# felixyu7/perceiver-io-1

Hardware: AMD Instinct MI355X
Metric: samples/sec (whole node) IMDB MLM seq_len=512 at 1/2/4/8 MI355X (higher is better)
Workload: dtype bf16; 1 GPU; mlm256; model=perceiver-io-mlm latents=256x64 layers=3x(1+6) vocab=10003, global_batch=64, seq_len=512, parallelism=dp1, backend=hip, graph=True, allreduce_in_graph=False, bucket_update=False

## Files before the change

### perceiver_io_amd/csrc/attention.hip

```cpp
#include "common.h"

namespace pio {

constexpr int KT = 64;

template <int D, int NWV>
__global__ __launch_bounds__(64 * NWV) void attn_fwd_kernel(AttnArgs a, uint16_t* __restrict__ O,
                                                            float* __restrict__ LSE, float* __restrict__ Opart,
                                                            float* __restrict__ MLpart, int nsplit,
                                                            int tiles_per_split) {
  constexpr int LDK = D + 8;
  constexpr int LDV = (D < 32 ? 32 : D) + 8;
  constexpr int NT = (D < 32) ? 1 : D / 32;
  constexpr int KS = D / 16;
  constexpr int CH = D / 8;
  constexpr int NTH = 64 * NWV;
  constexpr int NST0 = 4 * NTH / (KT * CH);
  constexpr int NST = NST0 >= 4 ? 4 : (NST0 >= 1 ? NST0 : 1);
  constexpr int NI = (NST * KT * CH + NTH - 1) / NTH;
  constexpr bool PF = NI <= 4;
  __shared__ __attribute__((aligned(16))) uint16_t sK[NST * KT * LDK];
  __shared__ __attribute__((aligned(16))) uint16_t sV[NST * KT * LDV + 64];

  const int w = wave_id(), l = lane_id(), r = l & 31, hh = l >> 5;
  const Blk3 blk = xcd_block3();
  const int h = blk.y;
  const int b = blk.z / nsplit, split = blk.z % nsplit;
  const int q0 = (blk.x * NWV + w) * 32;
  const int qi = q0 + r;
  const uint32_t dkey = a.drop_thresh ? drop_key(a.seedp, a.site, 2u) : 0u;
  const int qc = qi < a.Nq ? qi : a.Nq - 1;

  bf16x8 qf[KS];
  {
    const uint16_t* qp = a.q + (long long)b * a.q_bs + (long long)qc * a.q_rs + h * D + 8 * hh;
#pragma unroll
    for (int s = 0; s < KS; ++s) qf[s] = *reinterpret_cast<const bf16x8*>(qp + 16 * s);
  }

  const bool ones_den = D < 32 && !a.drop_thresh;
  if (D < 32) {
    const short pv = ones_den ? (short)0x3F80 : (short)0;
    const bf16x8 pad8 = {pv, pv, pv, pv, pv, pv, pv, pv};
    for (int i = threadIdx.x; i < NST * KT; i += NTH)
      *reinterpret_cast<bf16x8*>(sV + i * LDV + 16) = pad8, *reinterpret_cast<bf16x8*>(sV + i * LDV + 24) = pad8;
// ... 298 lines not shown
  bool kpad = false;
  if constexpr (KM) {
    const unsigned char* kmp = (a.kmask && kin) ? a.kmask + (long long)b * a.Nk + key
                                                : reinterpret_cast<const unsigned char*>(kZero32B);
    const unsigned char kmv = *kmp;
    kpad = (kmv != 0) | !kin;
  }

  const int HD = a.H * D;
  const bool vec_out = ((((uintptr_t)dq | (uintptr_t)dk | (uintptr_t)dv) & 15) == 0) &&
                       (((dq_bs | dk_bs | dv_bs) & 3) == 0) && (((dq_rs | dk_rs | dv_rs) & 3) == 0);
  const uint16_t* kbp = a.k + (long long)b * a.k_bs + h * D;
  const uint16_t* vbp = a.v + (long long)b * a.v_bs + h * D;
  const uint16_t* qbp = a.q + (long long)b * a.q_bs + h * D;
  const uint16_t* dobp = dO + (long long)b * a.Nq * HD + h * D;
  const int nqt_all = (a.Nq + 31) / 32;
  const int qt_begin = qsplit * q_tiles_per_split;
  const int nqt = min(nqt_all, qt_begin + q_tiles_per_split);

  bf16x8 qreg[NI];
  float lreg = 0.f;
  bool lq_out = false;
  auto fetch = [&](int qt0) {
    const int q00 = qt0 * 32;
#pragma unroll
    for (int i = 0; i < NI; ++i) {
      const int c = threadIdx.x + NTH * i, isdo = c >= NQS * 32 * CH, cc = isdo ? c - NQS * 32 * CH : c;
      const int qq = q00 + cc / CH, col = (cc % CH) * 8;
      const bool ok = c < NQS * 64 * CH && qq < a.Nq;
      const uint16_t* p = !ok ? reinterpret_cast<const uint16_t*>(kZero32B)
                              : (isdo ? dobp + (long long)qq * HD + col : qbp + (long long)qq * a.q_rs + col);
      qreg[i] = *reinterpret_cast<const bf16x8*>(p);
    }
    {
      const int t = threadIdx.x < NQS * 64 ? threadIdx.x : 0;
      const int isd = t >= NQS * 32, qq = q00 + (isd ? t - NQS * 32 : t);
      const long long idx = ((long long)b * a.Nq + qq) * a.H + h;
      const bool ok = qq < a.Nq;
      lreg = *(!ok ? kZero32B : (isd ? delta + idx : LSE + idx));
      lq_out = !ok && !isd;
    }
  };
  bf16x8 kf[KS], vf[KS];
#pragma unroll
  for (int s = 0; s < KS; ++s) {
    kf[s] = *reinterpret_cast<const bf16x8*>(kbp + (long long)kc * a.k_rs + 16 * s + 8 * hh);
    vf[s] = *reinterpret_cast<const bf16x8*>(vbp + (long long)kc * a.v_rs + 16 * s + 8 * hh);
  }
  fetch(qt_begin);
  if (D < 32) {
    for (int i = threadIdx.x; i < KB; i += NTH) {
      *reinterpret_cast<bf16x8*>(sK + i * LD + 16) = bf16x8{0, 0, 0, 0, 0, 0, 0, 0};
      *reinterpret_cast<bf16x8*>(sK + i * LD + 24) = bf16x8{0, 0, 0, 0, 0, 0, 0, 0};
// ... 110 lines not shown
    lds_sync();
    PIO_TS(4 + 4 * ((qt0 - qt_begin) / NQS));
    if constexpr (D == 16 && NW == 8 && (NQS == 4 || NQS == 2)) {
      const int j = w % NQS, mh = w / NQS, g = l >> 4;
      if (mh < 2 && qt0 + j < nqt) {
        const uint16_t* tS = sdS + j * KB * LDS_;
        f32x4 a0 = f32x4{0.f, 0.f, 0.f, 0.f}, a1 = f32x4{0.f, 0.f, 0.f, 0.f};
#pragma unroll
        for (int k0 = 0; k0 < KB; k0 += 64) {
          a0 = mfma16(frag16_tr(tS, LDS_, 16 * mh, k0), frag16_tr(sK, LD, 0, k0), a0);
          a1 = mfma16(frag16_tr(tS, LDS_, 16 * mh, k0 + 32), frag16_tr(sK, LD, 0, k0 + 32), a1);
        }
#pragma unroll
        for (int i = 0; i < 4; ++i) {
          const int qq = (qt0 + j) * 32 + 16 * mh + 4 * g + i;
          if (qq < a.Nq) {
            const long long di = (long long)b * dq_bs + (long long)qq * dq_rs + h * D + (l & 15);
            const float v = (a0[i] + a1[i]) * a.scale;
            if constexpr (OBF) reinterpret_cast<uint16_t*>(dq)[di] = f2bf(v);
            else if (dq_atomic) atomicAdd(dq + di, v);
            else dq[di] = v;
          }
        }
      }
    } else if (w < NQS && qt0 + w < nqt) {
      const uint16_t* tS = sdS + w * KB * LDS_;
#pragma unroll
      for (int t = 0; t < NT; ++t) {
        f32x16 dq_acc = f32x16{}, dq_acc2 = f32x16{};
#pragma unroll
        for (int k0 = 0; k0 < KB; k0 += 32) {
          dq_acc = mfma32(frag_ks(tS, LDS_, 0, k0), frag_ks(sK, LD, 32 * t, k0), dq_acc);
          dq_acc2 = mfma32(frag_ks(tS, LDS_, 0, k0 + 16), frag_ks(sK, LD, 32 * t, k0 + 16), dq_acc2);
        }
        dq_acc += dq_acc2;
        if (dq_atomic || !vec_out || D > 32) {
#pragma unroll
          for (int i = 0; i < 16; ++i) {
            const int dd = 32 * t + r, qq = (qt0 + w) * 32 + acc_row(i, hh);
            if (dd < D && qq < a.Nq) {
              float* dst = dq + (long long)b * dq_bs + (long long)qq * dq_rs + h * D + dd;
              const float v = dq_acc[i] * a.scale;
              if (dq_atomic) atomicAdd(dst, v);
              else *dst = v;
            }
          }
        } else {
          float* sE = reinterpret_cast<float*>(sdS + w * KB * LDS_);
          constexpr int LDE = D + 4;
#pragma unroll
          for (int i = 0; i < 16; ++i)
            if (r < D) sE[acc_row(i, hh) * LDE + r] = dq_acc[i] * a.scale;
          constexpr int CPR = D / 4;
#pragma unroll
          for (int c = l; c < 32 * CPR; c += 64) {
            const int qq = (qt0 + w) * 32 + c / CPR, col = (c % CPR) * 4;
            if (qq < a.Nq)
              *reinterpret_cast<float4*>(dq + (long long)b * dq_bs + (long long)qq * dq_rs + h * D + col) =
                  *reinterpret_cast<const float4*>(sE + (c / CPR) * LDE + col);
          }
        }
      }
    }
    PIO_TS(5 + 4 * ((qt0 - qt_begin) / NQS));
  }
  PIO_TS(40);
  if constexpr (D <= 32 && 2 * KB * (D + 4) * 4 <= NQS * KB * LDS_ * 2) {
    if (vec_out && nqs == 1) {
      constexpr int LDE = D + 4, CPR = D / 4;
      float* sE = reinterpret_cast<float*>(sdS);
      lds_sync();
#pragma unroll
// ... 295 lines not shown
```

### perceiver_io_amd/csrc/binding.cpp

```cpp
#include <torch/extension.h>
#include <ATen/hip/HIPContext.h>
#include <hip/hip_runtime.h>

#include "host_api.h"

#include <tuple>
#include <unordered_map>
#include <vector>

using torch::Tensor;
using OptT = c10::optional<Tensor>;

namespace {
hipStream_t stream() { return at::hip::getCurrentHIPStream(); }

#ifndef PIO_CHECKS
#define PIO_CHECKS 0
#endif
int64_t check_errors(bool reset) {
  return (int64_t)(pio::check_errors_elementwise(reset) | pio::check_errors_optim(reset) |
                   pio::check_errors_mlm_head(reset) | pio::check_errors_mlm_select(reset) |
                   pio::check_errors_ce_head(reset) | pio::check_errors_topk_head(reset) |
                   pio::check_errors_rowgemm(reset) | pio::check_errors_pixel_head(reset) |
                   pio::check_errors_soft_ce_head(reset) | pio::check_errors_augment(reset) |
// ... 78 lines not shown
    const Tensor& m = *kmask;
    CHECK_CUDA(m);
    TORCH_CHECK(m.scalar_type() == torch::kBool || m.scalar_type() == torch::kUInt8, "key mask must be bool/uint8");
    TORCH_CHECK(m.is_contiguous() && m.size(0) == a.B && m.size(1) == a.Nk, "key mask must be (B, Nk) contiguous");
    a.kmask = reinterpret_cast<const uint8_t*>(m.data_ptr());
  }
  a.scale = (float)scale;
  a.scale_log2 = (float)(scale * 1.4426950408889634);
  const pio::DropCfg d = make_drop(seed, site, dropout_p);
  a.drop_thresh = d.thresh;
  a.drop_scale = d.scale;
  a.seedp = d.seed;
  a.site = d.site;
  return a;
}
}

std::vector<Tensor> attn_fwd(Tensor q, Tensor k, Tensor v, OptT kmask, int64_t H, int64_t D, double scale,
                             double dropout_p, OptT seed, int64_t nsplit, int64_t site) {
  auto a = make_args(q, k, v, kmask, (int)H, (int)D, scale, dropout_p, seed, site);
  auto opts = q.options();
  Tensor O = torch::empty({a.B, a.Nq, H * D}, opts.dtype(torch::kBFloat16));
  Tensor L = torch::empty({a.B, a.Nq, H}, opts.dtype(torch::kFloat32));
  Tensor Op, ML;
  float* opp = nullptr; float* mlp = nullptr;
  if (nsplit > 1) {
    Op = torch::empty({nsplit, a.B, a.Nq, H, D}, opts.dtype(torch::kFloat32));
    ML = torch::empty({nsplit, a.B, a.Nq, H, 2}, opts.dtype(torch::kFloat32));
    opp = Op.data_ptr<float>(); mlp = ML.data_ptr<float>();
  }
  pio::attn_fwd_launch(a, (int)D, bfp_mut(O), L.data_ptr<float>(), opp, mlp, (int)std::max<int64_t>(1, nsplit), stream());
  return {O, L};
}

std::tuple<OptT, OptT> attn_weights(Tensor q, Tensor k, OptT kmask, Tensor lse, int64_t H, int64_t D, double scale,
// ... 15 lines not shown
    if (nchunks > 1) part = torch::empty({a.B, nchunks, a.Nk}, opts);
  }
  pio::attn_weights_launch(a, (int)D, f32p(lse), want_avg ? avg->data_ptr<float>() : nullptr,
                           want_mass ? mass->data_ptr<float>() : nullptr,
                           part.defined() ? part.data_ptr<float>() : nullptr, nchunks, stream());
  return {avg, mass};
}

namespace {
pio::SlabJob make_job(const OptT& slab, std::vector<Tensor>& dsts, const std::vector<int64_t>& offs);
}

std::vector<Tensor> attn_bwd(Tensor q, Tensor k, Tensor v, OptT kmask, Tensor o, Tensor dO, Tensor lse, OptT delta_in,
                             int64_t H, int64_t D, double scale, double dropout_p, OptT seed, OptT dq_out,
                             OptT dk_out, OptT dv_out, bool kv_accumulate, int64_t site, bool dq_zeroed,
                             bool kv_zeroed, OptT job_slab, std::vector<Tensor> job_dsts, std::vector<int64_t> job_offs) {
  auto a = make_args(q, k, v, kmask, (int)H, (int)D, scale, dropout_p, seed, site);
  const pio::SlabJob job = make_job(job_slab, job_dsts, job_offs);
  TORCH_CHECK(dO.is_contiguous() && o.is_contiguous(), "O / dO must be contiguous (B, Nq, H*D)");
  auto f32 = q.options().dtype(torch::kFloat32);
  if (dq_out.has_value() && dq_out->scalar_type() == torch::kBFloat16) {
    TORCH_CHECK(dk_out.has_value() && dv_out.has_value() && dk_out->scalar_type() == torch::kBFloat16 &&
                    dv_out->scalar_type() == torch::kBFloat16 && delta_in.has_value() && !kv_accumulate,
                "bf16 attn_bwd outputs: dq/dk/dv all bf16, delta given, no accumulation");
    Tensor dq = *dq_out, dk = *dk_out, dv = *dv_out;
    TORCH_CHECK(dq.stride(2) == 1 && dk.stride(2) == 1 && dv.stride(2) == 1, "dq/dk/dv need unit inner stride");
    Tensor delta = *delta_in;
    TORCH_CHECK(delta.is_contiguous() && delta.numel() == (int64_t)a.B * a.Nq * H, "delta must be (B, Nq, H)");
    CHECK_DT(delta, torch::kFloat32);
    if (pio::attn_bwd_bf16_ok(a, (int)D)) {
      pio::attn_bwd_bf16_launch(a, (int)D, bfp(dO), f32p(lse), delta.data_ptr<float>(), bfp_mut(dq), dq.stride(0),
                                (int)dq.stride(1), bfp_mut(dk), dk.stride(0), (int)dk.stride(1), bfp_mut(dv),
                                dv.stride(0), (int)dv.stride(1), job, stream());
    } else {
      if (job.slab) pio::slab_reduce_launch(job, stream());
      std::vector<Tensor> nd;
      auto r = attn_bwd(q, k, v, kmask, o, dO, lse, delta_in, H, D, scale, dropout_p, seed, c10::nullopt, c10::nullopt,
                        c10::nullopt, false, site, false, false, c10::nullopt, nd, {});
      dq.copy_(r[0]); dk.copy_(r[1]); dv.copy_(r[2]);
    }
    return {dq, dk, dv};
  }
  if (job.slab) pio::slab_reduce_launch(job, stream());
  Tensor dq = dq_out.has_value() ? *dq_out : torch::empty({a.B, a.Nq, H * D}, f32);
  Tensor dk = dk_out.has_value() ? *dk_out : torch::empty({a.B, a.Nk, H * D}, f32);
  Tensor dv = dv_out.has_value() ? *dv_out : torch::empty({a.B, a.Nk, H * D}, f32);
  TORCH_CHECK(dq.stride(2) == 1 && dk.stride(2) == 1 && dv.stride(2) == 1, "dq/dk/dv need unit inner stride");
  TORCH_CHECK(dq.size(0) == a.B && dq.stride(0) == a.Nq * dq.stride(1), "dq must be batch-dense");
  CHECK_DT(dq, torch::kFloat32); CHECK_DT(dk, torch::kFloat32); CHECK_DT(dv, torch::kFloat32);
  Tensor delta;
  if (delta_in.has_value()) {
    delta = *delta_in;
    TORCH_CHECK(delta.is_contiguous() && delta.numel() == (int64_t)a.B * a.Nq * H, "delta must be (B, Nq, H)");
    CHECK_DT(delta, torch::kFloat32);
  } else {
    delta = torch::empty({a.B, a.Nq, H}, f32);
  }
  auto rows3 = [](Tensor& t) { return pio::Rows3{t.data_ptr<float>(), t.stride(0), (int)t.stride(1)}; };
  pio::AttnBwdArgs b{};
  b.a = a;
  b.O = bfp(o);
  b.dO = bfp(dO);
  b.LSE = f32p(lse);
  b.delta = delta.data_ptr<float>();
// ... 888 lines not shown
  const int d = like.get_device();
  auto it = tickets.find(d);
  if (it == tickets.end()) it = tickets.emplace(d, torch::zeros({kCeTickets}, like.options().dtype(torch::kInt32))).first;
  return it->second;
}
constexpr int64_t kCeRowBlockTickets = 4096;
static Tensor& ce_rb_tickets(const Tensor& like) {
  static std::unordered_map<int, Tensor> tickets;
  const int d = like.get_device();
  auto it = tickets.find(d);
  if (it == tickets.end())
    it = tickets.emplace(d, torch::zeros({kCeRowBlockTickets}, like.options().dtype(torch::kInt32))).first;
  return it->second;
}

std::vector<Tensor> mlm_select(Tensor labels, int64_t cap, int64_t gcap, OptT sticky, OptT queries) {
  CHECK_DT(labels, torch::kInt64);
  TORCH_CHECK(labels.dim() == 2 && labels.is_contiguous(), "labels must be (B, L) contiguous");
  const int B = (int)labels.size(0), L = (int)labels.size(1);
  TORCH_CHECK(cap > 0 && cap <= L && gcap > 0 && B > 0, "bad capacities");
  auto i64 = labels.options();
  Tensor idx_b = torch::empty({B, cap}, i64), lab_b = torch::empty({B, cap}, i64);
  Tensor count = torch::empty({B}, i64.dtype(torch::kInt32));
  Tensor gidx = torch::empty({gcap}, i64), glab = torch::empty({gcap}, i64);
  Tensor total = torch::empty({1}, i64.dtype(torch::kFloat32)), ovf = torch::empty({1}, i64.dtype(torch::kBool));
  const float* P = nullptr;
  float* qp = nullptr;
  int C = 0;
  Tensor q;
  if (queries.has_value()) {
    CHECK_DT(*queries, torch::kFloat32);
    TORCH_CHECK(queries->dim() == 2 && queries->is_contiguous() && queries->size(0) >= L && queries->size(1) % 4 == 0 &&
                    queries->get_device() == labels.get_device(),
                "mlm_select: queries must be a contiguous fp32 (>= L, C) array, C % 4 == 0, on the labels' device");
    C = (int)queries->size(1);
    P = queries->data_ptr<float>();
    q = torch::empty({B, cap, C}, queries->options());
    qp = q.data_ptr<float>();
  }
  pio::mlm_select_launch(labels.data_ptr<int64_t>(), B, L, (int)cap, (int)gcap, idx_b.data_ptr<int64_t>(),
                         lab_b.data_ptr<int64_t>(), count.data_ptr<int>(), gidx.data_ptr<int64_t>(),
                         glab.data_ptr<int64_t>(), total.data_ptr<float>(), ovf.data_ptr<bool>(),
                         sticky.has_value() ? sticky->data_ptr<bool>() : nullptr, P, C, qp, stream());
  std::vector<Tensor> out{idx_b, lab_b, gidx, glab, total, ovf};
  if (queries.has_value()) out.push_back(q);
  return out;
}

static const int64_t* opt_idx(const OptT& idx, int64_t n) {
  if (!idx.has_value()) return nullptr;
  CHECK_DT(*idx, torch::kInt64);
  TORCH_CHECK(idx->is_contiguous() && idx->numel() == n, "ce: idx must hold one source row per row");
  return idx->data_ptr<int64_t>();
}

std::vector<Tensor> ce_fwd(Tensor h, OptT idx, Tensor labels, Tensor w, Tensor bias, Tensor count, OptT zero_out,
                           bool count_labels) {
  TORCH_CHECK(h.is_contiguous() && w.is_contiguous() && labels.is_contiguous() && bias.is_contiguous());
  CHECK_DT(labels, torch::kInt64);
  CHECK_DT(h, torch::kFloat32);
// ... 1220 lines not shown
  pio::attn_fwd_pe_launch(a, stream());
  pio::attn_combine_launch(a.Opart, a.MLpart, bfp_mut(o), lse.data_ptr<float>(), ns, (long long)B * Nq * H, 32, stream());
  return {o, lse};
}

void set_deterministic(bool on) { g_det = on; }
bool get_deterministic() { return g_det; }

PYBIND11_MODULE(TORCH_EXTENSION_NAME, m) {
  m.def("set_deterministic", &set_deterministic);
  m.def("check_errors", &check_errors, py::arg("reset") = true);
  m.def("checked_build", &checked_build);
  m.def("get_deterministic", &get_deterministic);
  m.doc() = "Perceiver IO CDNA4 (gfx950) kernels";
  m.def("attn_fwd", &attn_fwd, py::arg("q"), py::arg("k"), py::arg("v"), py::arg("kmask"), py::arg("H"), py::arg("D"),
        py::arg("scale"), py::arg("dropout_p"), py::arg("seed"), py::arg("nsplit"), py::arg("site") = 0);
  m.def("attn_bwd", &attn_bwd, py::arg("q"), py::arg("k"), py::arg("v"), py::arg("kmask"), py::arg("o"), py::arg("dO"),
        py::arg("lse"), py::arg("delta_in"), py::arg("H"), py::arg("D"), py::arg("scale"), py::arg("dropout_p"),
        py::arg("seed"), py::arg("dq_out"), py::arg("dk_out"), py::arg("dv_out"), py::arg("kv_accumulate") = false,
        py::arg("site") = 0, py::arg("dq_zeroed") = false, py::arg("kv_zeroed") = false,
        py::arg("job_slab") = py::none(), py::arg("job_dsts") = std::vector<Tensor>{},
        py::arg("job_offs") = std::vector<int64_t>{});
  m.def("attn_weights", &attn_weights, py::arg("q"), py::arg("k"), py::arg("kmask"), py::arg("lse"), py::arg("H"),
        py::arg("D"), py::arg("scale"), py::arg("want_avg"), py::arg("want_mass"));
  m.def("attn_bwd_zero_plan", &pio::attn_bwd_zero_plan, py::arg("B"), py::arg("H"), py::arg("Nq"), py::arg("Nk"),
        py::arg("D"));
  m.def("ln_linear_fwd", &ln_linear_fwd, py::arg("x"), py::arg("lnw"), py::arg("lnb"), py::arg("eps"), py::arg("w"),
        py::arg("bias"), py::arg("act"), py::arg("res"), py::arg("out_bf16"), py::arg("save_stats"),
        py::arg("pe") = py::none(), py::arg("kin") = -1, py::arg("pe_index") = py::none());
  m.def("post_attn_fwd", &post_attn_fwd, py::arg("o"), py::arg("x"), py::arg("wo"), py::arg("bo"), py::arg("g2"),
        py::arg("be2"), py::arg("eps"), py::arg("w1"), py::arg("b1"), py::arg("w2"), py::arg("b2"),
        py::arg("seed") = py::none(), py::arg("site") = 0, py::arg("p") = 0.0);
  m.def("sa_layer_fwd", &sa_layer_fwd, py::arg("qkv"), py::arg("x"), py::arg("N"), py::arg("scale"), py::arg("wo"),
        py::arg("bo"), py::arg("g2"), py::arg("be2"), py::arg("eps"), py::arg("w1"), py::arg("b1"), py::arg("w2"),
        py::arg("b2"), py::arg("lnw") = py::none(), py::arg("lnb") = py::none(), py::arg("wq") = py::none(),
        py::arg("bq") = py::none(), py::arg("seed") = py::none(), py::arg("site") = 0, py::arg("p") = 0.0);
  m.def("sb_fwd", &sb_fwd, py::arg("x"), py::arg("params"), py::arg("scale"), py::arg("eps"),
// ... 23 lines not shown
        py::arg("seed") = py::none(), py::arg("site") = 0, py::arg("p") = 0.0, py::arg("zero_out") = py::none());
  m.def("ln_linear_bwd", &ln_linear_bwd, py::arg("g"), py::arg("w"), py::arg("x"), py::arg("mean"), py::arg("rstd"),
        py::arg("lnw"), py::arg("lnb"), py::arg("dres"), py::arg("need_dx"), py::arg("dlnw"), py::arg("dlnb"),
        py::arg("dW"), py::arg("db"), py::arg("pe") = py::none(), py::arg("kin") = -1, py::arg("slab") = false,
        py::arg("job_slab") = py::none(), py::arg("job_dsts") = std::vector<Tensor>(),
        py::arg("job_offs") = std::vector<int64_t>(), py::arg("dx_out") = py::none(), py::arg("pe_index") = py::none());
  m.def("text_kv_fwd", &text_kv_fwd, py::arg("ids"), py::arg("E"), py::arg("P"), py::arg("scale"), py::arg("eps"),
        py::arg("la"), py::arg("lb"));
  m.def("text_kv_bwd", &text_kv_bwd, py::arg("ga"), py::arg("gb"), py::arg("x"), py::arg("mean"), py::arg("rstd"),
        py::arg("la"), py::arg("lb"), py::arg("grads"), py::arg("slab") = false, py::arg("job_slab") = py::none(),
        py::arg("job_dsts") = std::vector<Tensor>(), py::arg("job_offs") = std::vector<int64_t>());
  m.def("wgrad", &wgrad, py::arg("g"), py::arg("a"), py::arg("amode"), py::arg("mean"), py::arg("rstd"), py::arg("lnw"),
        py::arg("lnb"), py::arg("rows_per_wg"), py::arg("dW"), py::arg("db"), py::arg("pe") = py::none(),
        py::arg("kin") = -1, py::arg("pe_index") = py::none());
  m.def("mlm_select", &mlm_select, py::arg("labels"), py::arg("cap"), py::arg("gcap"), py::arg("sticky") = py::none(),
        py::arg("queries") = py::none());
  m.def("index_add_rows", &index_add_rows);
  m.def("gather_rows", &gather_rows, py::arg("src"), py::arg("idx"));
  m.def("batch_sum2", &batch_sum2, py::arg("a"), py::arg("b"), py::arg("ob_acc") = py::none());
  m.def("pixel_ce_fwd", &pixel_ce_fwd);
  m.def("pixel_ce_bwd", &pixel_ce_bwd);
  m.def("pixel_seg_fwd", &pixel_seg_fwd);
  m.def("pixel_seg_bwd", &pixel_seg_bwd);
  m.def("pixel_predict", &pixel_predict, py::arg("h"), py::arg("w"), py::arg("b"), py::arg("qidx"), py::arg("qvalid"),
        py::arg("Q"), py::arg("npix"), py::arg("labels") = py::none());
  m.def("nonzero_compact", &nonzero_compact, py::arg("img"), py::arg("cap"), py::arg("segs") = 0, py::arg("tile") = 0);
  m.def("event_compact", &event_compact, py::arg("img"), py::arg("lab"), py::arg("words"), py::arg("key_cap"),
        py::arg("query_cap"), py::arg("wmask"), py::arg("ncls"), py::arg("segs") = 0, py::arg("tile") = 0);
  m.def("stage_step", &stage_step, py::arg("dsts"), py::arg("srcs"), py::arg("hyper_dst") = py::none(),
        py::arg("hyper") = std::vector<double>{}, py::arg("seed_dst") = py::none(),
        py::arg("seeds") = std::vector<int64_t>{});
// ... 75 lines not shown
```

### perceiver_io_amd/csrc/host_api.h

```cpp
#pragma once
#include <stdint.h>

#include <hip/hip_runtime_api.h>

namespace pio {


struct AttnArgs {
  const uint16_t* q; long long q_bs; int q_rs;
  const uint16_t* k; long long k_bs; int k_rs;
  const uint16_t* v; long long v_bs; int v_rs;
  const uint8_t* kmask;
  int B, H, Nq, Nk;
  float scale_log2;
  float scale;
  uint32_t drop_thresh;
  float drop_scale;
  const int64_t* seedp;
  uint32_t site;
};

struct DropCfg {
  const int64_t* seed;
  uint32_t site;
  uint32_t thresh;
  float scale;
};

constexpr int kMaxSlabSegs = 16;
constexpr int kSlabColsPerBlock = 1024;
struct SlabJob {
  const float* slab;
  int S, P, nbx, nblk;
  int det;
// ... 423 lines not shown
```

### perceiver_io_amd/ops/emulation.py

```python
from __future__ import annotations

import math
import torch
import torch.nn.functional as F

LOG2E = 1.4426950408889634


def _bf(x):
    return x.to(torch.bfloat16).to(torch.float32)


M32 = 0xFFFFFFFF


def _u32(x):
    return x & M32


def hash3(a, b, c):
    h = _u32(_u32(a * 0x9E3779B1) ^ _u32(b + 0x7F4A7C15))
    h = h ^ _u32(c * 0x85EBCA77)
    h = _u32((h ^ (h >> 15)) * 0x2C1B3C6D)
    h = _u32((h ^ (h >> 12)) * 0x297A2D39)
# ... 246 lines not shown
def _qkv(q, k, v, H, D):
    B = max(q.shape[0], k.shape[0])
    qf = q[:, :, : H * D].float().expand(B, -1, -1).reshape(B, q.shape[1], H, D).permute(0, 2, 1, 3)
    kf = k[:, :, : H * D].float().reshape(B, k.shape[1], H, D).permute(0, 2, 1, 3)
    vf = v[:, :, : H * D].float().reshape(B, v.shape[1], H, D).permute(0, 2, 1, 3)
    return B, qf, kf, vf


def _scores(qf, kf, kmask, scale):
    s = torch.matmul(qf, kf.transpose(-1, -2)) * scale
    if kmask is not None:
        s = s.masked_fill(kmask.view(kmask.shape[0], 1, 1, -1).bool(), float("-inf"))
    return s


def attn_fwd(q, k, v, kmask, H, D, scale, dropout_p, seed, nsplit, site=0):
    B, qf, kf, vf = _qkv(q, k, v, H, D)
    s = _scores(qf, kf, kmask, scale)
    lse = torch.logsumexp(s, -1)
    p = torch.exp(s - lse[..., None])
    p = torch.nan_to_num(p, nan=0.0)
    if dropout_p > 0:
        p = p * attn_drop_mask(seed, site, B, H, q.shape[1], k.shape[1], dropout_p, q.device)
    o = torch.matmul(_bf(p), vf)
    lse2 = torch.where(torch.isfinite(lse), lse * LOG2E, torch.full_like(lse, float("inf")))
    o = o.permute(0, 2, 1, 3).reshape(B, q.shape[1], H * D).to(torch.bfloat16)
    return o, lse2.permute(0, 2, 1).contiguous()


def attn_weights(q, k, kmask, lse, H, D, scale, want_avg, want_mass):
    if not (want_avg or want_mass):
        raise ValueError("attn_weights: at least one of avg / mass must be requested")
    B, qf, kf, _ = _qkv(q, k, k, H, D)
    s = torch.matmul(qf, kf.transpose(-1, -2)) * scale
    if lse is not None:
        l2 = lse.float().permute(0, 2, 1).unsqueeze(-1)
        l2 = torch.where(torch.isfinite(l2), l2, torch.full_like(l2, float("inf")))
        p = torch.exp2(s * LOG2E - l2)
        if kmask is not None:
            p = p.masked_fill(kmask.view(B, 1, 1, -1).bool(), 0.0)
    else:
        if kmask is not None:
            s = s.masked_fill(kmask.view(B, 1, 1, -1).bool(), float("-inf"))
        p = torch.nan_to_num(torch.softmax(s, -1), nan=0.0)
    avg = p.sum(1) * (1.0 / H)
    return (avg if want_avg else None), (avg.sum(1) if want_mass else None)


def attn_bwd(q, k, v, kmask, o, dO, lse, delta_in, H, D, scale, dropout_p, seed, dq_out, dk_out, dv_out,
             kv_accumulate=False, site=0, dq_zeroed=False, kv_zeroed=False, job_slab=None, job_dsts=(), job_offs=()):
    _run_job(job_slab, job_dsts, job_offs)
    B, qf, kf, vf = _qkv(q, k, v, H, D)
    s = _scores(qf, kf, kmask, scale)
    l2 = lse.permute(0, 2, 1)
    p = torch.exp2(s * LOG2E - l2[..., None])
    p = torch.nan_to_num(p, nan=0.0)
    dof = dO.float().reshape(B, -1, H, D).permute(0, 2, 1, 3)
    if delta_in is not None:
        delta = delta_in.float().reshape(B, -1, H).permute(0, 2, 1)[..., None]
    else:
        of = o.float().reshape(B, -1, H, D).permute(0, 2, 1, 3)
        delta = (dof * of).sum(-1, keepdim=True)
    dp = torch.matmul(dof, vf.transpose(-1, -2))
    if dropout_p > 0:
        m = attn_drop_mask(seed, site, B, H, q.shape[1], k.shape[1], dropout_p, q.device)
        ds = p * (dp * m - delta)
        pd = p * m
    else:
        ds = p * (dp - delta)
        pd = p
    dq = torch.matmul(ds, kf) * scale
    dk = torch.matmul(ds.transpose(-1, -2), qf) * scale
    dv = torch.matmul(pd.transpose(-1, -2), dof)

    def merge(t):
        return t.permute(0, 2, 1, 3).reshape(B, t.shape[2], H * D)

# ... 118 lines not shown
        return d + dres if dres is not None else d
    return None


def wgrad(g, a, amode, mean, rstd, lnw, lnb, rows_per_wg, dW, db=None, pe=None, kin=-1, pe_index=None):
    af = _split_x(a, pe, kin if kin >= 0 else a.shape[1], pe_index)
    if amode == 1:
        af = (af - mean[:, None]) * rstd[:, None] * lnw + lnb
    elif amode == 2:
        af = F.gelu(af)
    _acc(dW, _bf(g.float()).t() @ _bf(af))
    if db is not None:
        _acc(db, g.float().sum(0))


def mlm_select(labels, cap, gcap, sticky=None, queries=None):
    B, L = labels.shape
    sel = labels != -100
    pos = torch.cumsum(sel.to(torch.int64), 1) - 1
    idx_b = (torch.arange(cap, device=labels.device) % L).repeat(B, 1)
    lab_b = torch.full((B, cap), -100, dtype=torch.int64, device=labels.device)
    keep = sel & (pos < cap)
    rows = torch.arange(B, device=labels.device)[:, None].expand(B, L)
    cols = torch.arange(L, device=labels.device).expand(B, L)
    idx_b[rows[keep], pos[keep]] = cols[keep]
    lab_b[rows[keep], pos[keep]] = labels[keep]
    count = sel.sum(1)
    n = count.clamp(max=cap)
    slot_ok = torch.arange(cap, device=labels.device)[None, :] < n[:, None]
    flat = torch.nonzero(slot_ok.reshape(-1)).reshape(-1)
    gidx = torch.zeros(gcap, dtype=torch.int64, device=labels.device)
    glab = torch.full((gcap,), -100, dtype=torch.int64, device=labels.device)
    m = min(gcap, flat.numel())
    gidx[:m] = flat[:m]
    glab[:m] = lab_b.reshape(-1)[flat[:m]]
    total = count.sum().float().reshape(1)
    ovf = ((count > cap).any() | (n.sum() > gcap)).reshape(1)
    if sticky is not None:
        sticky.logical_or_(ovf.reshape(sticky.shape))
    if queries is not None:
        return idx_b, lab_b, gidx, glab, total, ovf, queries.index_select(0, idx_b.reshape(-1)).view(B, cap, -1)
    return idx_b, lab_b, gidx, glab, total, ovf


def _ce_rows(h, idx):
    return h if idx is None else h.index_select(0, idx)


def ce_fwd(h, idx, labels, w, bias, count, zero_out=None, count_labels=False):
    if zero_out is not None:
        zero_out.zero_()
    if count_labels:
        count.reshape(-1)[0] = (labels >= 0).sum()
    logits = _bf(_ce_rows(h, idx).float()) @ _bf(w.float()).t() + bias
    lse = torch.logsumexp(logits, -1)
    valid = labels >= 0
    picked = logits.gather(1, labels.clamp(min=0)[:, None])[:, 0]
# ... 939 lines not shown
```

### perceiver_io_amd/ops/fused.py

```python
from __future__ import annotations

import math
import os
from dataclasses import dataclass
from typing import List, Optional

import torch

from . import emulation, ext
from ..parallel.reducer import bucket_ready_point

EPS = 1e-5
WGRAD_SLAB = True
BF16_DQKV = True
ATTN_SLAB = True
CHAIN_ATT = True
TALL_ROWS = 1 << 17


def kernels(t: torch.Tensor):
    return ext.require() if t.is_cuda else emulation


class WeightCache:
# ... 363 lines not shown
        C, H = spec.C, spec.heads
        D = C // H
        scale = 1.0 / math.sqrt(D)
        wq, wkv, wo, w1, w2 = bw
        if spec.cross:
            g_q, b_q, g_kv, b_kv = ps[0:4]
            rest = ps[5:] if spec.packed else ps[7:]
        else:
            g_q, b_q = ps[0:2]
            rest = ps[3:]
        bin_, _, bo, g2, be2, _, b1, _, b2 = rest
        Bq, Nq = x_q.shape[0], x_q.shape[1]
        xq2 = x_q.reshape(Bq * Nq, C)
        if not xq2.is_contiguous():
            xq2 = xq2.contiguous()
        if spec.cross:
            B, M = x_kv.shape[0], x_kv.shape[1]
            xkv2 = x_kv.reshape(B * M, x_kv.shape[2])
            hq = _LOOKAHEAD["have_q"]
            if hq is not None and hq[4] is g_q and hq[0].data_ptr() == xq2.data_ptr() and hq[0].numel() == xq2.numel():
                q, mean_q, rstd_q = hq[1:4]
                _LOOKAHEAD["have_q"] = None
                ctx.q_handoff = True
            else:
                q, mean_q, rstd_q = K.ln_linear_fwd(xq2, g_q, b_q, EPS, wq, bin_[:C], 0, None, True, True)
            key = id(ps[0])
            ent = src.entries.get(key) if src is not None else None
            ctx.kv_owner = ent is None or bool(ent.pop("claim", False))
            if ent is None:
                kv_sb = False
# ... 39 lines not shown
                k3, v3 = kv3[:, :, :C], kv3[:, :, C:]
        else:
            B = Bq
            qkv, mean_q, rstd_q = K.ln_linear_fwd(xq2, g_q, b_q, EPS, wq, bin_, 0, None, True, True)
            qkv3 = qkv.view(B, Nq, 3 * C)
            q3, k3, v3 = qkv3[:, :, :C], qkv3[:, :, C:2 * C], qkv3[:, :, 2 * C:]
            xkv2 = kv = mean_kv = rstd_kv = None
        from .attention import pick_splits

        imp = ent.get("implicit") if spec.cross else None
        if imp is not None:
            P, pes, pesq, wt, kin = imp
            o, lse = K.attn_fwd_pe(q3, P, xkv2, pes, pesq, wt, H, scale, kin, EPS, 0)
        else:
            nsplit = pick_splits(B, H, Nq, k3.shape[1], p_attn > 0)
            o, lse = K.attn_fwd(q3, k3, v3, kmask, H, D, scale, p_attn, seed, nsplit)
        o2 = o.view(B * Nq, C)
        nxt, _LOOKAHEAD["want"] = _LOOKAHEAD["want"], None
        want_pa, _LOOKAHEAD["want_pa"] = _LOOKAHEAD["want_pa"], None
        if (want_pa and spec.cross and nxt is None and p_attn == 0.0 and Nq == 32 and H == 4 and Bq in (1, B)
                and o2.is_contiguous()):
            z = torch.empty((B * Nq, C), device=o2.device, dtype=torch.float32)
            _LOOKAHEAD["have_pa"] = dict(key=z.data_ptr(), ctx=ctx, pre=[o2, xq2, wo, bo, g2, be2, w1, b1, w2, b2],
                                         ps=(rest[1], bo, g2, be2, rest[5], b1, rest[7], b2))
            ctx.pa_key = z.data_ptr()
            y = m2 = r2 = u = torch.empty(0, device=o2.device)
        elif nxt is not None and spec.cross:
            z, y, m2, r2, u, qkv_n, mean_n, rstd_n = K.post_attn_ln_linear_fwd(
                o2, xq2, wo, bo, g2, be2, EPS, w1, b1, w2, b2, nxt[0], nxt[1], nxt[2], nxt[3], seed=seed, p=p_attn)
            _LOOKAHEAD["have"] = (z, qkv_n, mean_n, rstd_n, nxt[0])
            ctx.lookahead_z = z.data_ptr()
# ... 117 lines not shown
                if imp is not None:
                    P, pes, pesq, wt, kin = imp
                    K.attn_bwd_pe_implicit(qx, P, pes, pesq, wt, do.view(B, Nq, C), lse, delta3, xkv2, dq, ent["pe_D"],
                                           ent["pe_part"], H, scale, kin, EPS, acc, ent["pe_bsplit"],
                                           dq_zeroed=dq_pre is not None, d_zeroed=d_pre is not None)
                else:
                    K.attn_bwd_pe(qx, kv, do.view(B, Nq, C), lse, delta3, mean_kv, rstd_kv, xkv2, dq, ent["pe_D"],
                                  ent["pe_part"], H, scale, acc, ent["pe_bsplit"], dq_zeroed=dq_pre is not None,
                                  d_zeroed=d_pre is not None)
            else:
                acc = ent["dkv"] is not None
                kv_pre = not acc and d_pre is not None and d_pre.dim() == 3
                if not acc:
                    ent["dkv"] = d_pre if kv_pre else torch.empty((B, M, 2 * C), **f32)
                dkv = ent["dkv"]
                dq, _, _ = K.attn_bwd(qx, kv3[:, :, :C], kv3[:, :, C:], kmask, o, do.view(B, Nq, C), lse, delta3, H,
                                      D, scale, ctx.p_attn, ctx.seed, dq_pre, dkv[:, :, :C], dkv[:, :, C:], acc,
                                      dq_zeroed=dq_pre is not None, kv_zeroed=kv_pre)
            leaf_g = None
            if ctx.q_leaf is not None and Bq == 1 and B > 1 and not getattr(ctx, "q_handoff", False):
                leaf_g = _grad_of(ctx.q_leaf)
                if leaf_g is not None and not (leaf_g.is_contiguous() and leaf_g.data_ptr() % 16 == 0):
                    leaf_g = None
            if Bq == 1 and B > 1 and dq.shape[0] == B:
                dq2, dres = K.batch_sum2(dq.contiguous(), dy.view(B, Nq, C), ob_acc=leaf_g)
            elif Bq == 1 and B > 1:
                dq2 = dq.reshape(Nq, C)
                _, dres = K.batch_sum2(None, dy.view(B, Nq, C).contiguous(), ob_acc=leaf_g)
            else:
                dq2, dres = dq.reshape(B * Nq, C), dy
            q_out = dict(dx_out=dres.view(Nq, C)) if leaf_g is not None else {}
            Ckv = g_kv.shape[0]
            Rq = dq2.shape[0]
# ... 300 lines not shown
                sl.defer(K, ll_dsts(P[i]) + pa_dsts(P[i - 1]))
            elif getattr(ctx, "handoff", None) is not None:
                _LOOKAHEAD["bwd"] = dict(key=ctx.handoff, g=dqkv.view(R, 3 * C), wq=bws[0][0], x=xl, mean1=mean1,
                                         rstd1=rstd1, lnw=P[0][0], lnb=P[0][1], dres=dy, ll_dsts=ll_dsts(P[0]))
                dx = dy
            else:
                sl = _GradSlab(R, LL_SIZES(C), dz2)
                dx = K.ln_linear_bwd(dqkv.view(R, 3 * C), bws[0][0], xl, mean1, rstd1, P[0][0], P[0][1], dy, True,
                                     *sl.targets(), slab=True, **_take_job())
                sl.defer(K, ll_dsts(P[0]))
        return (None, None, None, None, dx.view(B, N, C)) + (None,) * len(ps)


_LOOKAHEAD = {"want": None, "have": None, "bwd": None, "want_q": None, "have_q": None, "bwd_q": None,
              "want_pa": None, "have_pa": None, "bwd_pa": None,
              "want_kv": None}


def _sa_block_plan(block, rows: int):
    layers = list(block)
    specs, pss = [], []
    for layer in layers:
        spec, ps = layer_spec_and_params(layer)
        specs.append(spec)
        pss.append(ps)
    ok = (WGRAD_SLAB and len(layers) > 1 and all(_fusable(lay) for lay in layers)
          and all(sp == specs[0] for sp in specs) and specs[0].C in SA_BLOCK_CHANNELS and not specs[0].cross
          and rows < TALL_ROWS)
    return layers, specs, pss, ok


# ... 479 lines not shown
```

### perceiver_io_amd/ops/mlm_head.py

```python
from __future__ import annotations

import math

import torch
import torch.nn.functional as F

from . import ext

_overflow = None
_flags = {}


def last_overflow():
    return _overflow


def overflow_flag(device) -> torch.Tensor:
    device = torch.device(device)
    f = _flags.get(device)
    if f is None:
        f = _flags[device] = torch.zeros((), dtype=torch.bool, device=device)
    return f


# ... 206 lines not shown
            return kernels(param).gather_rows(param.detach(), idx.contiguous())
        return param.index_select(0, idx)

    @staticmethod
    def backward(ctx, g):
        (idx,) = ctx.saved_tensors
        if ctx.needs_input_grad[0]:
            _index_add_grad(ctx.param, idx, g)
        return None, None


class _SelectQueries(torch.autograd.Function):

    @staticmethod
    def forward(ctx, param, labels, cap, gcap, sticky):
        idx, _, gidx, glab, total, ovf, q = ext.require().mlm_select(labels.contiguous(), cap, gcap, sticky,
                                                                     param.detach().contiguous())
        ctx.save_for_backward(idx)
        ctx.param = param
        ctx.mark_non_differentiable(idx, gidx, glab, total, ovf)
        ctx.set_materialize_grads(False)
        return q, idx, gidx, glab, total, ovf

    @staticmethod
    def backward(ctx, g, *_):
        (idx,) = ctx.saved_tensors
        if g is not None and ctx.needs_input_grad[0]:
            _index_add_grad(ctx.param, idx.reshape(-1), g)
        return None, None, None, None, None


def masked_decode_loss(decoder, x_latent: torch.Tensor, labels: torch.Tensor, p: float = 0.15, clump: float = 1.0):
    from ..parallel.reducer import bucket_ready_point
    from . import use_hip

    x_latent = bucket_ready_point(x_latent, decoder, "decoder")
    B, L = labels.shape
    decoder.check_latent(x_latent)
    lin = decoder.output_adapter.linear
    cap = row_capacity(L, p, clump)
    if use_hip(x_latent) and lin.weight.shape[1] in (32, 64, 128):
        q, idx, gidx, glab, total, ovf = _SelectQueries.apply(decoder.output, labels, cap, capacity(B * L, p, clump),
                                                              overflow_flag(labels.device).view(1))
        global _overflow
        _overflow = ovf
        h = decoder.cross_attention(q, x_latent)
        return _MaskedCE.apply(h, lin.weight, lin.bias, gidx, glab, total)
    idx, labels_c, count = compact_per_row(labels, cap)
    q = _GatherQueries.apply(decoder.output, idx.reshape(-1)).view(B, cap, -1)
    h = decoder.cross_attention(q, x_latent)
    return compact_lm_loss(h, labels_c, count, lin.weight, lin.bias, B * L, p, clump)


def classification_loss(decoder, x_latent: torch.Tensor, labels: torch.Tensor):
    from . import use_hip

    h = decoder.hidden(x_latent)
    ad = decoder.output_adapter
    lin = getattr(ad, "linear", None)
    if (lin is not None and use_hip(h) and h.dim() == 3 and h.shape[1] == 1 and h.shape[-1] in (32, 64, 128)
            and labels.dim() == 1 and labels.shape[0] == h.shape[0]):
# ... 72 lines not shown
```

Baseline: 48900 samples/s.

## Skip padded MLM decoder query tiles using per-sample masked-token counts

Passes the per-row count of selected MLM query positions from mlm_select into the decoder cross-attention forward and backward kernels. Forward blocks whose query tile lies entirely beyond the live count write zeros and infinite LSE and exit early. Backward clamps the query-tile loop to the live count and zeroes dq up front. This cuts attention work on padded capacity rows, at the cost of an extra dq memset and restricting the path to non-deterministic, single-split, fp32-dq configurations.

Result: no change. 48920 samples/s (median of 2 runs) (+0.0%).

```diff
diff --git a/perceiver_io_amd/csrc/attention.hip b/perceiver_io_amd/csrc/attention.hip
--- a/perceiver_io_amd/csrc/attention.hip
+++ b/perceiver_io_amd/csrc/attention.hip
@@ -29,6 +29,23 @@
   const int q0 = (blk.x * NWV + w) * 32;
   const int qi = q0 + r;
   const uint32_t dkey = a.drop_thresh ? drop_key(a.seedp, a.site, 2u) : 0u;
+  if (a.nq_dev != nullptr && nsplit == 1) {
+    const int nq = min(a.nq_dev[b], a.Nq);
+    if ((int)blk.x * NWV * 32 >= nq) {
+      if (qi < a.Nq) {
+        uint16_t* op = O + ((long long)b * a.Nq + qi) * (a.H * D) + h * D;
+#pragma unroll
+        for (int t2 = 0; t2 < NT; ++t2)
+#pragma unroll
+          for (int g = 0; g < 4; ++g) {
+            const int dd = 32 * t2 + 8 * g + 4 * hh;
+            if (dd < D) *reinterpret_cast<uint2*>(op + dd) = make_uint2(0u, 0u);
+          }
+        if (hh == 0) LSE[((long long)b * a.Nq + qi) * a.H + h] = INFINITY;
+      }
+      return;
+    }
+  }
   const int qc = qi < a.Nq ? qi : a.Nq - 1;
 
   bf16x8 qf[KS];
@@ -357,7 +374,8 @@
   const uint16_t* vbp = a.v + (long long)b * a.v_bs + h * D;
   const uint16_t* qbp = a.q + (long long)b * a.q_bs + h * D;
   const uint16_t* dobp = dO + (long long)b * a.Nq * HD + h * D;
-  const int nqt_all = (a.Nq + 31) / 32;
+  const int nq = a.nq_dev != nullptr ? min(a.nq_dev[b], a.Nq) : a.Nq;
+  const int nqt_all = (nq + 31) / 32;
   const int qt_begin = qsplit * q_tiles_per_split;
   const int nqt = min(nqt_all, qt_begin + q_tiles_per_split);
 
@@ -370,7 +388,7 @@
     for (int i = 0; i < NI; ++i) {
       const int c = threadIdx.x + NTH * i, isdo = c >= NQS * 32 * CH, cc = isdo ? c - NQS * 32 * CH : c;
       const int qq = q00 + cc / CH, col = (cc % CH) * 8;
-      const bool ok = c < NQS * 64 * CH && qq < a.Nq;
+      const bool ok = c < NQS * 64 * CH && qq < nq;
       const uint16_t* p = !ok ? reinterpret_cast<const uint16_t*>(kZero32B)
                               : (isdo ? dobp + (long long)qq * HD + col : qbp + (long long)qq * a.q_rs + col);
       qreg[i] = *reinterpret_cast<const bf16x8*>(p);
@@ -379,7 +397,7 @@
       const int t = threadIdx.x < NQS * 64 ? threadIdx.x : 0;
       const int isd = t >= NQS * 32, qq = q00 + (isd ? t - NQS * 32 : t);
       const long long idx = ((long long)b * a.Nq + qq) * a.H + h;
-      const bool ok = qq < a.Nq;
+      const bool ok = qq < nq;
       lreg = *(!ok ? kZero32B : (isd ? delta + idx : LSE + idx));
       lq_out = !ok && !isd;
     }
@@ -520,7 +538,7 @@
 #pragma unroll
         for (int i = 0; i < 4; ++i) {
           const int qq = (qt0 + j) * 32 + 16 * mh + 4 * g + i;
-          if (qq < a.Nq) {
+          if (qq < nq) {
             const long long di = (long long)b * dq_bs + (long long)qq * dq_rs + h * D + (l & 15);
             const float v = (a0[i] + a1[i]) * a.scale;
             if constexpr (OBF) reinterpret_cast<uint16_t*>(dq)[di] = f2bf(v);
@@ -544,7 +562,7 @@
 #pragma unroll
           for (int i = 0; i < 16; ++i) {
             const int dd = 32 * t + r, qq = (qt0 + w) * 32 + acc_row(i, hh);
-            if (dd < D && qq < a.Nq) {
+            if (dd < D && qq < nq) {
               float* dst = dq + (long long)b * dq_bs + (long long)qq * dq_rs + h * D + dd;
               const float v = dq_acc[i] * a.scale;
               if (dq_atomic) atomicAdd(dst, v);
@@ -561,7 +579,7 @@
 #pragma unroll
           for (int c = l; c < 32 * CPR; c += 64) {
             const int qq = (qt0 + w) * 32 + c / CPR, col = (c % CPR) * 4;
-            if (qq < a.Nq)
+            if (qq < nq)
               *reinterpret_cast<float4*>(dq + (long long)b * dq_bs + (long long)qq * dq_rs + h * D + col) =
                   *reinterpret_cast<const float4*>(sE + (c / CPR) * LDE + col);
           }
diff --git a/perceiver_io_amd/csrc/binding.cpp b/perceiver_io_amd/csrc/binding.cpp
--- a/perceiver_io_amd/csrc/binding.cpp
+++ b/perceiver_io_amd/csrc/binding.cpp
@@ -116,11 +116,21 @@
   a.site = d.site;
   return a;
 }
+
+const int* nq_ptr(const OptT& nq, const pio::AttnArgs& a, const Tensor& q) {
+  if (!nq.has_value()) return nullptr;
+  CHECK_CUDA(*nq);
+  CHECK_DT(*nq, torch::kInt32);
+  TORCH_CHECK(nq->is_contiguous() && nq->numel() == a.B && nq->get_device() == q.get_device() && q.size(0) == a.B,
+              "nq must be (B,) int32 on the queries' device, with per-sample queries");
+  return nq->data_ptr<int>();
+}
 }
 
 std::vector<Tensor> attn_fwd(Tensor q, Tensor k, Tensor v, OptT kmask, int64_t H, int64_t D, double scale,
-                             double dropout_p, OptT seed, int64_t nsplit, int64_t site) {
+                             double dropout_p, OptT seed, int64_t nsplit, int64_t site, OptT nq) {
   auto a = make_args(q, k, v, kmask, (int)H, (int)D, scale, dropout_p, seed, site);
+  a.nq_dev = nq_ptr(nq, a, q);
   auto opts = q.options();
   Tensor O = torch::empty({a.B, a.Nq, H * D}, opts.dtype(torch::kBFloat16));
   Tensor L = torch::empty({a.B, a.Nq, H}, opts.dtype(torch::kFloat32));
@@ -166,8 +176,13 @@
 std::vector<Tensor> attn_bwd(Tensor q, Tensor k, Tensor v, OptT kmask, Tensor o, Tensor dO, Tensor lse, OptT delta_in,
                              int64_t H, int64_t D, double scale, double dropout_p, OptT seed, OptT dq_out,
                              OptT dk_out, OptT dv_out, bool kv_accumulate, int64_t site, bool dq_zeroed,
-                             bool kv_zeroed, OptT job_slab, std::vector<Tensor> job_dsts, std::vector<int64_t> job_offs) {
+                             bool kv_zeroed, OptT job_slab, std::vector<Tensor> job_dsts, std::vector<int64_t> job_offs,
+                             OptT nq) {
   auto a = make_args(q, k, v, kmask, (int)H, (int)D, scale, dropout_p, seed, site);
+  a.nq_dev = nq_ptr(nq, a, q);
+  TORCH_CHECK(a.nq_dev == nullptr || (!g_det && !(dq_out.has_value() && dq_out->scalar_type() == torch::kBFloat16) &&
+                                      !(D == 128 && a.Nq == 1)),
+              "attn_bwd: nq needs fp32 outputs, more than one query and non-deterministic mode");
   const pio::SlabJob job = make_job(job_slab, job_dsts, job_offs);
   TORCH_CHECK(dO.is_contiguous() && o.is_contiguous(), "O / dO must be contiguous (B, Nq, H*D)");
   auto f32 = q.options().dtype(torch::kFloat32);
@@ -188,7 +203,7 @@
       if (job.slab) pio::slab_reduce_launch(job, stream());
       std::vector<Tensor> nd;
       auto r = attn_bwd(q, k, v, kmask, o, dO, lse, delta_in, H, D, scale, dropout_p, seed, c10::nullopt, c10::nullopt,
-                        c10::nullopt, false, site, false, false, c10::nullopt, nd, {});
+                        c10::nullopt, false, site, false, false, c10::nullopt, nd, {}, c10::nullopt);
       dq.copy_(r[0]); dk.copy_(r[1]); dv.copy_(r[2]);
     }
     return {dq, dk, dv};
@@ -200,6 +215,10 @@
   TORCH_CHECK(dq.stride(2) == 1 && dk.stride(2) == 1 && dv.stride(2) == 1, "dq/dk/dv need unit inner stride");
   TORCH_CHECK(dq.size(0) == a.B && dq.stride(0) == a.Nq * dq.stride(1), "dq must be batch-dense");
   CHECK_DT(dq, torch::kFloat32); CHECK_DT(dk, torch::kFloat32); CHECK_DT(dv, torch::kFloat32);
+  if (a.nq_dev != nullptr && !dq_zeroed) {
+    dq.zero_();
+    dq_zeroed = true;
+  }
   Tensor delta;
   if (delta_in.has_value()) {
     delta = *delta_in;
@@ -1118,7 +1137,7 @@
   return it->second;
 }
 
-std::vector<Tensor> mlm_select(Tensor labels, int64_t cap, int64_t gcap, OptT sticky, OptT queries) {
+std::vector<Tensor> mlm_select(Tensor labels, int64_t cap, int64_t gcap, OptT sticky, OptT queries, bool want_count) {
   CHECK_DT(labels, torch::kInt64);
   TORCH_CHECK(labels.dim() == 2 && labels.is_contiguous(), "labels must be (B, L) contiguous");
   const int B = (int)labels.size(0), L = (int)labels.size(1);
@@ -1148,6 +1167,7 @@
                          sticky.has_value() ? sticky->data_ptr<bool>() : nullptr, P, C, qp, stream());
   std::vector<Tensor> out{idx_b, lab_b, gidx, glab, total, ovf};
   if (queries.has_value()) out.push_back(q);
+  if (want_count) out.push_back(count);
   return out;
 }
 
@@ -2398,13 +2418,14 @@
   m.def("get_deterministic", &get_deterministic);
   m.doc() = "Perceiver IO CDNA4 (gfx950) kernels";
   m.def("attn_fwd", &attn_fwd, py::arg("q"), py::arg("k"), py::arg("v"), py::arg("kmask"), py::arg("H"), py::arg("D"),
-        py::arg("scale"), py::arg("dropout_p"), py::arg("seed"), py::arg("nsplit"), py::arg("site") = 0);
+        py::arg("scale"), py::arg("dropout_p"), py::arg("seed"), py::arg("nsplit"), py::arg("site") = 0,
+        py::arg("nq") = py::none());
   m.def("attn_bwd", &attn_bwd, py::arg("q"), py::arg("k"), py::arg("v"), py::arg("kmask"), py::arg("o"), py::arg("dO"),
         py::arg("lse"), py::arg("delta_in"), py::arg("H"), py::arg("D"), py::arg("scale"), py::arg("dropout_p"),
         py::arg("seed"), py::arg("dq_out"), py::arg("dk_out"), py::arg("dv_out"), py::arg("kv_accumulate") = false,
         py::arg("site") = 0, py::arg("dq_zeroed") = false, py::arg("kv_zeroed") = false,
         py::arg("job_slab") = py::none(), py::arg("job_dsts") = std::vector<Tensor>{},
-        py::arg("job_offs") = std::vector<int64_t>{});
+        py::arg("job_offs") = std::vector<int64_t>{}, py::arg("nq") = py::none());
   m.def("attn_weights", &attn_weights, py::arg("q"), py::arg("k"), py::arg("kmask"), py::arg("lse"), py::arg("H"),
         py::arg("D"), py::arg("scale"), py::arg("want_avg"), py::arg("want_mass"));
   m.def("attn_bwd_zero_plan", &pio::attn_bwd_zero_plan, py::arg("B"), py::arg("H"), py::arg("Nq"), py::arg("Nk"),
@@ -2458,7 +2479,7 @@
         py::arg("lnb"), py::arg("rows_per_wg"), py::arg("dW"), py::arg("db"), py::arg("pe") = py::none(),
         py::arg("kin") = -1, py::arg("pe_index") = py::none());
   m.def("mlm_select", &mlm_select, py::arg("labels"), py::arg("cap"), py::arg("gcap"), py::arg("sticky") = py::none(),
-        py::arg("queries") = py::none());
+        py::arg("queries") = py::none(), py::arg("want_count") = false);
   m.def("index_add_rows", &index_add_rows);
   m.def("gather_rows", &gather_rows, py::arg("src"), py::arg("idx"));
   m.def("batch_sum2", &batch_sum2, py::arg("a"), py::arg("b"), py::arg("ob_acc") = py::none());
diff --git a/perceiver_io_amd/csrc/host_api.h b/perceiver_io_amd/csrc/host_api.h
--- a/perceiver_io_amd/csrc/host_api.h
+++ b/perceiver_io_amd/csrc/host_api.h
@@ -18,6 +18,7 @@
   float drop_scale;
   const int64_t* seedp;
   uint32_t site;
+  const int* nq_dev;
 };
 
 struct DropCfg {
diff --git a/perceiver_io_amd/ops/emulation.py b/perceiver_io_amd/ops/emulation.py
--- a/perceiver_io_amd/ops/emulation.py
+++ b/perceiver_io_amd/ops/emulation.py
@@ -284,7 +284,11 @@
     return s
 
 
-def attn_fwd(q, k, v, kmask, H, D, scale, dropout_p, seed, nsplit, site=0):
+def _nq_rows(nq, Nq, device):
+    return torch.arange(Nq, device=device)[None, :] < nq.to(torch.int64).clamp(max=Nq)[:, None]
+
+
+def attn_fwd(q, k, v, kmask, H, D, scale, dropout_p, seed, nsplit, site=0, nq=None):
     B, qf, kf, vf = _qkv(q, k, v, H, D)
     s = _scores(qf, kf, kmask, scale)
     lse = torch.logsumexp(s, -1)
@@ -295,7 +299,15 @@
     o = torch.matmul(_bf(p), vf)
     lse2 = torch.where(torch.isfinite(lse), lse * LOG2E, torch.full_like(lse, float("inf")))
     o = o.permute(0, 2, 1, 3).reshape(B, q.shape[1], H * D).to(torch.bfloat16)
-    return o, lse2.permute(0, 2, 1).contiguous()
+    lse2 = lse2.permute(0, 2, 1).contiguous()
+    if nq is not None and nsplit <= 1:
+        Nq = q.shape[1]
+        tile = 32 if Nq <= 32 else (64 if Nq <= 64 else 128)
+        first = torch.arange(Nq, device=q.device) // tile * tile
+        dead = first[None, :] >= nq.to(torch.int64).clamp(max=Nq)[:, None]
+        o = o.masked_fill(dead[:, :, None], 0.0)
+        lse2 = lse2.masked_fill(dead[:, :, None], float("inf"))
+    return o, lse2
 
 
 def attn_weights(q, k, kmask, lse, H, D, scale, want_avg, want_mass):
@@ -318,9 +330,16 @@
 
 
 def attn_bwd(q, k, v, kmask, o, dO, lse, delta_in, H, D, scale, dropout_p, seed, dq_out, dk_out, dv_out,
-             kv_accumulate=False, site=0, dq_zeroed=False, kv_zeroed=False, job_slab=None, job_dsts=(), job_offs=()):
+             kv_accumulate=False, site=0, dq_zeroed=False, kv_zeroed=False, job_slab=None, job_dsts=(), job_offs=(),
+             nq=None):
     _run_job(job_slab, job_dsts, job_offs)
     B, qf, kf, vf = _qkv(q, k, v, H, D)
+    live = None
+    if nq is not None:
+        live = _nq_rows(nq, q.shape[1], q.device)
+        qf = torch.where(live[:, None, :, None], qf, torch.zeros_like(qf))
+        lse = torch.where(live[:, :, None], lse, torch.full_like(lse, float("inf")))
+        dO = torch.where(live[:, :, None], dO, torch.zeros_like(dO))
     s = _scores(qf, kf, kmask, scale)
     l2 = lse.permute(0, 2, 1)
     p = torch.exp2(s * LOG2E - l2[..., None])
@@ -331,6 +350,8 @@
     else:
         of = o.float().reshape(B, -1, H, D).permute(0, 2, 1, 3)
         delta = (dof * of).sum(-1, keepdim=True)
+    if live is not None:
+        delta = torch.where(live[:, None, :, None], delta, torch.zeros_like(delta))
     dp = torch.matmul(dof, vf.transpose(-1, -2))
     if dropout_p > 0:
         m = attn_drop_mask(seed, site, B, H, q.shape[1], k.shape[1], dropout_p, q.device)
@@ -479,7 +500,7 @@
         _acc(db, g.float().sum(0))
 
 
-def mlm_select(labels, cap, gcap, sticky=None, queries=None):
+def mlm_select(labels, cap, gcap, sticky=None, queries=None, want_count=False):
     B, L = labels.shape
     sel = labels != -100
     pos = torch.cumsum(sel.to(torch.int64), 1) - 1
@@ -503,9 +524,12 @@
     ovf = ((count > cap).any() | (n.sum() > gcap)).reshape(1)
     if sticky is not None:
         sticky.logical_or_(ovf.reshape(sticky.shape))
+    out = (idx_b, lab_b, gidx, glab, total, ovf)
     if queries is not None:
-        return idx_b, lab_b, gidx, glab, total, ovf, queries.index_select(0, idx_b.reshape(-1)).view(B, cap, -1)
-    return idx_b, lab_b, gidx, glab, total, ovf
+        out += (queries.index_select(0, idx_b.reshape(-1)).view(B, cap, -1),)
+    if want_count:
+        out += (count.to(torch.int32),)
+    return out
 
 
 def _ce_rows(h, idx):
diff --git a/perceiver_io_amd/ops/fused.py b/perceiver_io_amd/ops/fused.py
--- a/perceiver_io_amd/ops/fused.py
+++ b/perceiver_io_amd/ops/fused.py
@@ -401,6 +401,8 @@
         xq2 = x_q.reshape(Bq * Nq, C)
         if not xq2.is_contiguous():
             xq2 = xq2.contiguous()
+        nq, _LOOKAHEAD["nq"] = _LOOKAHEAD["nq"], None
+        ctx.nq = None
         if spec.cross:
             B, M = x_kv.shape[0], x_kv.shape[1]
             xkv2 = x_kv.reshape(B * M, x_kv.shape[2])
@@ -470,7 +472,11 @@
             o, lse = K.attn_fwd_pe(q3, P, xkv2, pes, pesq, wt, H, scale, kin, EPS, 0)
         else:
             nsplit = pick_splits(B, H, Nq, k3.shape[1], p_attn > 0)
-            o, lse = K.attn_fwd(q3, k3, v3, kmask, H, D, scale, p_attn, seed, nsplit)
+            if nq is not None and spec.cross and Bq == B and nq.numel() == B and nsplit == 1:
+                ctx.nq = nq
+                o, lse = K.attn_fwd(q3, k3, v3, kmask, H, D, scale, p_attn, seed, nsplit, nq=nq)
+            else:
+                o, lse = K.attn_fwd(q3, k3, v3, kmask, H, D, scale, p_attn, seed, nsplit)
         o2 = o.view(B * Nq, C)
         nxt, _LOOKAHEAD["want"] = _LOOKAHEAD["want"], None
         want_pa, _LOOKAHEAD["want_pa"] = _LOOKAHEAD["want_pa"], None
@@ -618,9 +624,10 @@
                 if not acc:
                     ent["dkv"] = d_pre if kv_pre else torch.empty((B, M, 2 * C), **f32)
                 dkv = ent["dkv"]
+                nqk = dict(nq=ctx.nq) if ctx.nq is not None and dq_pre is not None else {}
                 dq, _, _ = K.attn_bwd(qx, kv3[:, :, :C], kv3[:, :, C:], kmask, o, do.view(B, Nq, C), lse, delta3, H,
                                       D, scale, ctx.p_attn, ctx.seed, dq_pre, dkv[:, :, :C], dkv[:, :, C:], acc,
-                                      dq_zeroed=dq_pre is not None, kv_zeroed=kv_pre)
+                                      dq_zeroed=dq_pre is not None, kv_zeroed=kv_pre, **nqk)
             leaf_g = None
             if ctx.q_leaf is not None and Bq == 1 and B > 1 and not getattr(ctx, "q_handoff", False):
                 leaf_g = _grad_of(ctx.q_leaf)
@@ -951,7 +958,7 @@
 
 _LOOKAHEAD = {"want": None, "have": None, "bwd": None, "want_q": None, "have_q": None, "bwd_q": None,
               "want_pa": None, "have_pa": None, "bwd_pa": None,
-              "want_kv": None}
+              "want_kv": None, "nq": None}
 
 
 def _sa_block_plan(block, rows: int):
diff --git a/perceiver_io_amd/ops/mlm_head.py b/perceiver_io_amd/ops/mlm_head.py
--- a/perceiver_io_amd/ops/mlm_head.py
+++ b/perceiver_io_amd/ops/mlm_head.py
@@ -1,11 +1,14 @@
 from __future__ import annotations
 
 import math
+import os
 
 import torch
 import torch.nn.functional as F
 
 from . import ext
+
+COMPACT_DECODE = os.environ.get("PERCEIVER_MLM_COMPACT_DECODE", "1") != "0"
 
 _overflow = None
 _flags = {}
@@ -244,13 +247,13 @@
 
     @staticmethod
     def forward(ctx, param, labels, cap, gcap, sticky):
-        idx, _, gidx, glab, total, ovf, q = ext.require().mlm_select(labels.contiguous(), cap, gcap, sticky,
-                                                                     param.detach().contiguous())
+        idx, _, gidx, glab, total, ovf, q, count = ext.require().mlm_select(labels.contiguous(), cap, gcap, sticky,
+                                                                            param.detach().contiguous(), True)
         ctx.save_for_backward(idx)
         ctx.param = param
-        ctx.mark_non_differentiable(idx, gidx, glab, total, ovf)
+        ctx.mark_non_differentiable(idx, gidx, glab, total, ovf, count)
         ctx.set_materialize_grads(False)
-        return q, idx, gidx, glab, total, ovf
+        return q, idx, gidx, glab, total, ovf, count
 
     @staticmethod
     def backward(ctx, g, *_):
@@ -270,11 +273,19 @@
     lin = decoder.output_adapter.linear
     cap = row_capacity(L, p, clump)
     if use_hip(x_latent) and lin.weight.shape[1] in (32, 64, 128):
-        q, idx, gidx, glab, total, ovf = _SelectQueries.apply(decoder.output, labels, cap, capacity(B * L, p, clump),
-                                                              overflow_flag(labels.device).view(1))
+        q, idx, gidx, glab, total, ovf, count = _SelectQueries.apply(decoder.output, labels, cap,
+                                                                     capacity(B * L, p, clump),
+                                                                     overflow_flag(labels.device).view(1))
         global _overflow
         _overflow = ovf
-        h = decoder.cross_attention(q, x_latent)
+        from . import deterministic, fused
+
+        if COMPACT_DECODE and not deterministic():
+            fused._LOOKAHEAD["nq"] = count
+        try:
+            h = decoder.cross_attention(q, x_latent)
+        finally:
+            fused._LOOKAHEAD["nq"] = None
         return _MaskedCE.apply(h, lin.weight, lin.bias, gidx, glab, total)
     idx, labels_c, count = compact_per_row(labels, cap)
     q = _GatherQueries.apply(decoder.output, idx.reshape(-1)).view(B, cap, -1)
```
